# HydrogenSulfate/LFT

Measured on AMD Instinct MI355X. Metric: LF patches/sec (5x5 angRes, 32x32 LR, 4xSR), higher is better.
Workload: dtype bf16

## Files before the change

### lft_amd/_lib.py

```python
from __future__ import annotations

import ctypes
import os
import subprocess
from ctypes import POINTER, c_char_p, c_float, c_int, c_longlong, c_size_t, c_void_p

HERE = os.path.dirname(os.path.abspath(__file__))
CSRC = os.path.join(HERE, "csrc")
LIB_PATH = os.environ.get("LFT_LIB_PATH") or os.path.join(HERE, "liblft_hip.so")
SOURCES = ["lft_api.hip", "lft_common.cuh", "lft_kernels_a.cuh", "lft_kernels_b.cuh", "lft_train.cuh", "lft_train_host.cuh", "lft_metrics.cuh"]
ABI_VERSION = 5
STATUS_NONFINITE = 1001

PREC_F32, PREC_BF16, PREC_F16 = 0, 1, 2
MATH_F32, MATH_BF16X3, MATH_BF16X6 = 0, 1, 2
NUM_PARAMS = 78

_lib = None


class LftError(RuntimeError):
    pass


# ... 78 lines not shown
    "lft_spa_block_fwd": (c_int, [c_void_p, c_int, c_void_p, c_void_p, c_void_p, c_void_p, c_int, c_int, c_int, c_int, c_int, c_int, c_void_p]),
    "lft_upsample_fwd": (c_int, [c_void_p, c_void_p, c_void_p, c_void_p, c_void_p, c_int, c_int, c_int, c_int, c_int, c_int, c_void_p]),
    "lft_scene_counts": (c_int, [c_int, c_int, c_int, c_int, POINTER(c_int), POINTER(c_int)]),
    "lft_scene_divide": (c_int, [c_void_p, c_void_p, c_int, c_int, c_int, c_int, c_int, c_void_p]),
    "lft_scene_integrate": (c_int, [c_void_p, c_void_p, c_int, c_int, c_int, c_int, c_int, c_int, c_void_p]),
    "lft_train_tape_bytes": (c_int, [c_int, c_int, c_int, c_int, c_int, POINTER(c_size_t)]),
    "lft_train_grad_floats": (c_int, [c_int, POINTER(c_size_t)]),
    "lft_train_tape_offset": (c_int, [c_char_p, c_int, c_int, c_int, c_int, c_int, POINTER(c_size_t)]),
    "lft_train_forward": (c_int, [POINTER(c_void_p), c_int, c_void_p, c_void_p, c_void_p, c_int, c_int, c_int, c_int, c_int, c_int, c_void_p]),
    "lft_train_backward": (c_int, [POINTER(c_void_p), c_int, c_void_p, c_void_p, c_void_p, c_void_p, c_int, c_int, c_int, c_int, c_int, c_int, c_void_p]),
    "lft_train_backward_buckets": (c_int, [POINTER(c_void_p), c_int, c_void_p, c_void_p, c_void_p, c_void_p, c_int, c_int, c_int, c_int, c_int, c_int,
                                           c_void_p, c_void_p, c_void_p]),
    "lft_train_block_backward": (c_int, [POINTER(c_void_p), c_int, c_void_p, c_void_p, c_int, c_int, c_void_p, c_void_p, c_void_p,
                                         c_int, c_int, c_int, c_int, c_int, c_int, c_void_p]),
    "lft_train_grad_bucket": (c_int, [c_int, c_int, POINTER(c_size_t), POINTER(c_size_t)]),
    "lft_train_step_profiled": (c_int, [POINTER(c_void_p), c_int, c_void_p, c_void_p, c_void_p, c_void_p, c_void_p, c_int, c_int, c_int, c_int, c_int, c_int,
                                        c_void_p, c_int, POINTER(c_float), POINTER(c_char_p), POINTER(c_int)]),
    "lft_l1_loss": (c_int, [c_void_p, c_void_p, c_longlong, c_void_p, c_float, c_void_p, c_void_p, c_void_p]),
    "lft_adam_step": (c_int, [c_void_p, c_void_p, c_void_p, c_void_p, c_longlong, c_float, c_float, c_float, c_float, c_int, c_float, c_float, c_void_p]),
    "lft_view_metrics_scratch_bytes": (c_int, [c_int, c_int, c_int, c_int, POINTER(c_size_t)]),
    "lft_view_metrics": (c_int, [c_void_p, c_void_p, c_int, c_int, c_int, c_int, c_float, c_void_p, c_void_p, c_void_p, c_void_p]),
    "lft_debug_conv64": (c_int, [c_void_p, c_int, c_int, c_void_p, c_void_p, c_void_p, c_int, c_int, c_int, c_int, c_int, c_int, c_int, c_void_p]),
    "lft_mfma_selftest": (c_int, [c_void_p, c_void_p, c_void_p, c_void_p, c_void_p, c_int, c_void_p]),
}
EXPORTS = tuple(_SIGS)
TEST_EXPORTS = ("lft_debug_conv64", "lft_mfma_selftest")
BLOCK_UPSAMPLE, BLOCK_SPA, BLOCK_ANG, BLOCK_INIT = 0, 1, 2, 3
GRAD_BUCKETS = 3
BUCKET_FN = ctypes.CFUNCTYPE(c_int, c_void_p, c_int, c_size_t, c_size_t)


def lib() -> ctypes.CDLL:
    global _lib
    if _lib is None:
        if not os.path.exists(LIB_PATH):
            raise LftError(f"{LIB_PATH} is missing: the HIP extension has not been built "
                           "(run __graft_entry__.build()); there is no CPU fallback")
        L = ctypes.CDLL(LIB_PATH)
        L.lft_version.restype, L.lft_version.argtypes = c_int, []
        got = L.lft_version()
        if got != ABI_VERSION and not (os.environ.get("LFT_AB_ANY_ABI") == "1" and os.environ.get("LFT_LIB_PATH")):
            raise LftError(f"{LIB_PATH} reports ABI version {got}, this binding needs {ABI_VERSION}: rebuild it (__graft_entry__.build())")
        for name, (res, args) in _SIGS.items():
            if not hasattr(L, name) and got != ABI_VERSION:
                continue
            fn = getattr(L, name)
            fn.restype, fn.argtypes = res, args
        _lib = L
    return _lib
# ... 19 lines not shown
```

### lft_amd/csrc/lft_api.hip

```cpp
#include "../../include/lft_hip.h"
#include "../../include/lft_hip_test.h"
#include <hip/hip_runtime.h>
#include <stdint.h>

#include <cstdarg>
#include <cstdio>
#include <cmath>
#include <set>
#include <string>
#include <algorithm>
#include <utility>
#include <vector>

#ifndef LFT_TU
#define LFT_TU 0
#endif

namespace {
#include "lft_kernels_a.cuh"
#include "lft_kernels_b.cuh"
#include "lft_metrics.cuh"
#include "lft_train.cuh"
}

// ... 63 lines not shown
struct Dims {
    int B, A, V, h, w, hw, s, gp, gt, nchunk;
    long long ntok;
};

int make_dims(int B, int A, int h, int w, int s, int prec, Dims* d) {
    if (prec != LFT_PREC_F32 && prec != LFT_PREC_BF16 && prec != LFT_PREC_F16)
        return fail(LFT_ERR_ARG, "prec must be LFT_PREC_F32, LFT_PREC_BF16 or LFT_PREC_F16, got %d", prec);
    if (B < 1 || A < 1 || h < 1 || w < 1) return fail(LFT_ERR_SHAPE, "B, A, h, w must be positive (B=%d A=%d h=%d w=%d)", B, A, h, w);
    if (s != 2 && s != 4) return fail(LFT_ERR_SHAPE, "scale factor must be 2 or 4, got %d", s);
    if (A * A > 128) return fail(LFT_ERR_UNSUPPORTED, "angRes %d (A*A=%d views > 128) is not implemented in this build", A, A * A);
    if ((long long)B * A * A * h * w > (1LL << 27)) return fail(LFT_ERR_SHAPE, "too many tokens");
    d->B = B; d->A = A; d->V = A * A; d->h = h; d->w = w; d->hw = h * w; d->s = s;
    d->gp = (s + 2) * (s + 2); d->gt = (d->gp + 31) / 32; d->nchunk = 2 * s * s;
    d->ntok = (long long)B * d->V * d->hw;
    return 0;
}

constexpr int kFragsConv = 72, kFragsAng = 64, kFragsSpa1 = 240, kFragsSpa1NoQ = 208, kFragsSpa2 = 176;
inline int frags_up(const Dims& d) { return d.nchunk * (4 + 2 * d.gt); }

struct PackedLayout {
    size_t conv0_w, ln_ang[kLayers], ln_spa[kLayers], ang_pe, petok[kLayers], spa_pe_img;
    size_t s_conv[3], s_ang[kLayers], s_spa1[kLayers], s_spa2[kLayers], s_up, total;
};

PackedLayout packed_layout(const Dims& d, int prec) {
    const size_t esz = prec == LFT_PREC_F32 ? 4 : 2, fragb = 64 * 8 * esz;
    PackedLayout L;
    size_t o = 0;
    auto take = [&](size_t bytes) { size_t r = o; o = align256(o + bytes); return r; };
    L.conv0_w = take(576 * 4);
    for (int l = 0; l < kLayers; ++l) { L.ln_ang[l] = take(256 * 4); L.ln_spa[l] = take(512 * 4); }
    L.ang_pe = take((size_t)((d.V + 31) / 32) * 2048 * 4);
    for (int l = 0; l < kLayers; ++l) L.petok[l] = take((size_t)((d.hw + 32 * kNwSpa1 - 1) / (32 * kNwSpa1)) * kNwSpa1 * 4096 * esz);
    L.spa_pe_img = take((size_t)d.hw * 64 * esz);
    for (int i = 0; i < 3; ++i) L.s_conv[i] = take(kFragsConv * fragb);
    for (int l = 0; l < kLayers; ++l) {
        L.s_ang[l] = take(kFragsAng * fragb);
        L.s_spa1[l] = take(kFragsSpa1 * fragb);
        L.s_spa2[l] = take(kFragsSpa2 * fragb);
    }
    L.s_up = take((size_t)frags_up(d) * fragb);
    L.total = o;
    return L;
}

struct WorkLayout {
    size_t x0, feat, xa, xb, tok, q, k, v, o, g, status, total;
};
WorkLayout work_layout(const Dims& d, int prec) {
    const size_t esz = prec == LFT_PREC_F32 ? 4 : 2;
    WorkLayout W;
    size_t o = 0;
    auto take = [&](size_t bytes) { size_t r = o; o = align256(o + bytes); return r; };
    const size_t n = (size_t)d.ntok;
    W.x0 = take(n * 64 * esz); W.feat = take(n * 64 * esz); W.xa = take(n * 64 * esz); W.xb = take(n * 64 * esz);
    W.tok = take(n * 128 * esz); W.q = take(n * 128 * esz); W.k = take(n * 128 * esz); W.v = take(n * 128 * esz);
    W.o = take(n * 128 * esz);
    W.g = take(n * d.gp * 4);
    W.status = take(256);
    W.total = o;
    return W;
}

template <typename T> size_t lds_conv64(int w) { return WRing<T, kConv64Chunk, kNwConv>::LDS_BYTES + ConvIn<T, kNwConv>::bytes(w) + kNwConv * TileIO<2, T>::BYTES + kConvZeroRow; }
// ... 134 lines not shown
        {
            std::vector<PackOp> ops;
            ops.push_back(lin_op(q[4], 0, 128, 128, 0, 8, (sizeof(T) == 2 && tok_lane_major<T>(d)) ? 1 : 0, 1.0f));
            for (int c = 0; c < 4; ++c) {
                ops.push_back(lin_op(q[7], 64 * c, 64, 128, 0, 8, 1, 1.0f));
                ops.push_back(lin_op(q[8], 0, 128, 256, 64 * c, 4, 1, 1.0f));
            }
            ops.push_back(lin_op(q[9], 0, 64, 128, 0, 8, 1, 1.0f));
            if ((rc = run_pack<T>(ops, at<T>(packed, L.s_spa2[l]), kFragsSpa2, st))) return rc;
        }
        if ((rc = launch_spa1<T, true>((unsigned)((d.hw + 32 * kNwSpa1 - 1) / (32 * kNwSpa1)), at<T>(packed, L.spa_pe_img), at<T>(packed, L.s_spa1[l]), nullptr, nullptr,
                                       nullptr, nullptr, nullptr, nullptr, at<T>(packed, L.petok[l]), 1, d, st, nullptr))) return rc;
        LFT_LAUNCH_OK("k_spa1<pe>");
    }
    {
        std::vector<PackOp> ops;
        for (int c = 0; c < d.nchunk; ++c) {
            ops.push_back(lin_op(P[76], 32 * c, 32, 64, 0, 4, 1, 1.0f));
            PackOp m = lin_op(P[77], 0, d.gp, 0, 32 * c, 2, 1, 1.0f);
            m.kind = 1; m.s = d.s; m.ntiles = d.gt;
            ops.push_back(m);
        }
        if ((rc = run_pack<T>(ops, at<T>(packed, L.s_up), frags_up(d), st))) return rc;
    }
    return 0;
}

void launch_assemble(const float* lr, const float* g, float* out, int B, int A, int h, int w, int s, hipStream_t st, int gld = 0, unsigned* status = nullptr) {
    const dim3 tg((unsigned)((A * w + 7) / 8) * (unsigned)((A * h + 7) / 8) * (unsigned)B);
    if (!gld) gld = (s + 2) * (s + 2);
    if (s == 2) k_assemble_t<2><<<tg, 256, 0, st>>>(lr, g, out, B, A, h, w, gld, status);
    else k_assemble_t<4><<<tg, 256, 0, st>>>(lr, g, out, B, A, h, w, gld, status);
}

template <typename T>
int init_features(const void* packed, const PackedLayout& L, const float* lr, T* x0, T* ta, T* tb, T* feat, const Dims& d, hipStream_t st) {
    const int nimg = d.B * d.V, nwg = nimg * ((d.hw + 32 * kNwConv - 1) / (32 * kNwConv));
    const size_t lds = lds_conv64<T>(d.w);
    int rc;
    if ((rc = allow_lds(k_conv64<T, false>, lds, "k_conv64"))) return rc;
    if ((rc = allow_lds(k_conv64<T, true>, lds, "k_conv64"))) return rc;
    k_conv0<T><<<dim3((unsigned)((d.hw + kConv0Tok - 1) / kConv0Tok), (unsigned)nimg), 256, 0, st>>>(lr, at<float>(packed, L.conv0_w), x0, d.B, d.A, d.h, d.w);
    LFT_LAUNCH_OK("k_conv0");
    k_conv64<T, false><<<nwg, 64 * kNwConv, lds, st>>>(x0, ta, nullptr, at<T>(packed, L.s_conv[0]), nimg, d.h, d.w);
    LFT_LAUNCH_OK("k_conv64");
    k_conv64<T, false><<<nwg, 64 * kNwConv, lds, st>>>(ta, tb, nullptr, at<T>(packed, L.s_conv[1]), nimg, d.h, d.w);
// ... 90 lines not shown
    LFT_LAUNCH_OK("k_spa_attn");
    const unsigned nb = blocks_for(d.ntok, 32 * kNwSpa2);
    const bool lm = tok_lane_major<T>(d);
#define LFT_LAUNCH_SPA2(SKV, LMV, YLV)                                                                                      \
    do {                                                                                                                    \
        if ((rc = allow_lds(k_spa2<T, SKV, LMV, YLV>, lds_spa2<T>(), "k_spa2"))) return rc;                                 \
        k_spa2<T, SKV, LMV, YLV><<<nb, 64 * kNwSpa2, lds_spa2<T>(), st>>>(tok, o, at<T>(packed, L.s_spa2[l]), ln, skip, out, d.ntok, at<unsigned>(ws, W.status)); \
    } while (0)
    if (out_lm && !(skip && lm)) return fail(LFT_ERR_ARG, "internal: lane-major output needs the skip variant and full tiles");
    if (skip) { if (out_lm) LFT_LAUNCH_SPA2(true, true, true); else if (lm) LFT_LAUNCH_SPA2(true, true, false); else LFT_LAUNCH_SPA2(true, false, false); }
    else { if (lm) LFT_LAUNCH_SPA2(false, true, false); else LFT_LAUNCH_SPA2(false, false, false); }
#undef LFT_LAUNCH_SPA2
    LFT_LAUNCH_OK("k_spa2");
    return 0;
    }
}
template <typename T>
int spa_block(const void* packed, const PackedLayout& L, int l, const T* in, const T* skip, T* out, void* ws, const WorkLayout& W,
              const Dims& d, hipStream_t st, bool out_lm = false) {
    int rc;
    if ((rc = spa_part_a<T>(packed, L, l, in, ws, W, d, st))) return rc;
    return spa_part_b<T>(packed, L, l, skip, out, ws, W, d, st, out_lm);
}
template <typename T>
int upsample(const void* packed, const PackedLayout& L, const T* body, const float* lr, float* out, void* ws, const WorkLayout& W,
             const Dims& d, hipStream_t st, bool in_lm = false) {
    float* g = at<float>(ws, W.g);
    const unsigned nb = blocks_for(d.ntok, 32 * kNwUp);
    int rc;
#define LFT_LAUNCH_UP(GTV, LMV)                                                                                              \
    do {                                                                                                                    \
        if ((rc = allow_lds(k_up<T, GTV, LMV>, lds_up<T>(), "k_up"))) return rc;                                            \
        k_up<T, GTV, LMV><<<nb, 64 * kNwUp, lds_up<T>(), st>>>(body, at<T>(packed, L.s_up), g, d.ntok, d.nchunk, d.gp);     \
    } while (0)
    if (d.gt == 1) { if (in_lm) LFT_LAUNCH_UP(1, true); else LFT_LAUNCH_UP(1, false); }
    else { if (in_lm) LFT_LAUNCH_UP(2, true); else LFT_LAUNCH_UP(2, false); }
#undef LFT_LAUNCH_UP
    LFT_LAUNCH_OK("k_up");
    launch_assemble(lr, g, out, d.B, d.A, d.h, d.w, d.s, st, 0, at<unsigned>(ws, W.status));
    LFT_LAUNCH_OK("k_assemble");
    return 0;
}

template <typename T>
int forward_impl(const void* packed, const float* lr, float* out, void* ws, const Dims& d, int prec, hipStream_t st) {
    const PackedLayout L = packed_layout(d, prec);
    const WorkLayout W = work_layout(d, prec);
    T *x0 = at<T>(ws, W.x0), *feat = at<T>(ws, W.feat), *xa = at<T>(ws, W.xa), *xb = at<T>(ws, W.xb);
    int rc;
    if ((rc = init_features<T>(packed, L, lr, x0, xa, xb, feat, d, st))) return rc;
    const T* cur = feat;
    for (int l = 0; l < kLayers; ++l) {
        if ((rc = ang_block<T>(packed, L, l, cur, xa, d, st, at<unsigned>(ws, W.status)))) return rc;
        const bool last = l == kLayers - 1;
        if ((rc = spa_block<T>(packed, L, l, xa, last ? feat : nullptr, xb, ws, W, d, st, last && LFT_YLM && tok_lane_major<T>(d)))) return rc;
        cur = xb;
    }
    return upsample<T>(packed, L, xb, lr, out, ws, W, d, st, LFT_YLM && tok_lane_major<T>(d));
}

template <typename T>
int kernel_time_impl(const char* name, const void* packed, void* ws, const Dims& d, int prec, int reps, hipStream_t st, float* ms_out) {
    const PackedLayout L = packed_layout(d, prec);
    const WorkLayout W = work_layout(d, prec);
    T *x0 = at<T>(ws, W.x0), *feat = at<T>(ws, W.feat), *xa = at<T>(ws, W.xa), *xb = at<T>(ws, W.xb);
    const std::string k(name);
    auto once = [&]() -> int {
        if (k == "k_ang") return ang_block<T>(packed, L, 1, xb, xa, d, st, at<unsigned>(ws, W.status));
        if (k == "k_spa1") return spa_part_a<T>(packed, L, 1, xa, ws, W, d, st);
        if (k == "k_spa_b" || k == "k_spa_attn+k_spa2") return spa_part_b<T>(packed, L, 1, nullptr, xb, ws, W, d, st);
        if (k == "k_conv64") {
            const int nimg = d.B * d.V, nwg = nimg * ((d.hw + 32 * kNwConv - 1) / (32 * kNwConv));
            const size_t lds = lds_conv64<T>(d.w);
            int rc;
            if ((rc = allow_lds(k_conv64<T, false>, lds, "k_conv64"))) return rc;
            k_conv64<T, false><<<nwg, 64 * kNwConv, lds, st>>>(x0, feat, nullptr, at<T>(packed, L.s_conv[0]), nimg, d.h, d.w);
            LFT_LAUNCH_OK("k_conv64");
            return 0;
        }
        return fail(LFT_ERR_ARG, "lft_kernel_time: unknown kernel %s", name);
    };
    int rc;
    if ((rc = once())) return rc;
    hipEvent_t e0, e1;
    LFT_HIP_OK(hipEventCreate(&e0));
    LFT_HIP_OK(hipEventCreate(&e1));
    LFT_HIP_OK(hipEventRecord(e0, st));
    for (int i = 0; i < reps && !rc; ++i) rc = once();
    LFT_HIP_OK(hipEventRecord(e1, st));
    LFT_HIP_OK(hipEventSynchronize(e1));
    float ms = 0.0f;
    LFT_HIP_OK(hipEventElapsedTime(&ms, e0, e1));
    (void)hipEventDestroy(e0); (void)hipEventDestroy(e1);
// ... 134 lines not shown
}

int lft_spa_block_fwd(const void* packed, int layer, const void* act_in, const void* skip, void* act_out, void* workspace, int B, int A,
                      int h, int w, int s, int prec, void* stream) {
    Dims d; int rc;
    if (!packed || !act_in || !act_out || !workspace) return fail(LFT_ERR_ARG, "null pointer");
    if (layer < 0 || layer >= kLayers) return fail(LFT_ERR_ARG, "layer %d out of range", layer);
    if ((rc = make_dims(B, A, h, w, s, prec, &d))) return rc;
    const PackedLayout L = packed_layout(d, prec);
    const WorkLayout W = work_layout(d, prec);
    hipStream_t st = static_cast<hipStream_t>(stream);
    return LFT_BY_PREC(prec, spa_block<T>(packed, L, layer, static_cast<const T*>(act_in), static_cast<const T*>(skip),
                                          static_cast<T*>(act_out), workspace, W, d, st));
}

int lft_upsample_fwd(const void* packed, const void* act_in, const float* lr, float* out, void* workspace, int B, int A, int h, int w,
                     int s, int prec, void* stream) {
    Dims d; int rc;
    if (!packed || !act_in || !lr || !out || !workspace) return fail(LFT_ERR_ARG, "null pointer");
    if ((rc = make_dims(B, A, h, w, s, prec, &d))) return rc;
    const PackedLayout L = packed_layout(d, prec);
    const WorkLayout W = work_layout(d, prec);
    hipStream_t st = static_cast<hipStream_t>(stream);
    return LFT_BY_PREC(prec, upsample<T>(packed, L, static_cast<const T*>(act_in), lr, out, workspace, W, d, st));
}

int lft_debug_conv64(const void* packed, int which, int with_res, const void* in, const void* res, void* out, int B, int A, int h,
                     int w, int s, int prec, int extra_lds, void* stream) {
    Dims d; int rc;
    if (!packed || !in || !out || which < 0 || which > 2) return fail(LFT_ERR_ARG, "bad argument");
    if ((rc = make_dims(B, A, h, w, s, prec, &d))) return rc;
    const PackedLayout L = packed_layout(d, prec);
    hipStream_t st = static_cast<hipStream_t>(stream);
    const int nimg = d.B * d.V, nwg = nimg * ((d.hw + 32 * kNwConv - 1) / (32 * kNwConv));
    rc = LFT_BY_PREC(prec, [&]() -> int {
        const size_t lds = lds_conv64<T>(d.w) + extra_lds;
        int r;
        if ((r = allow_lds(k_conv64<T, false>, lds, "k_conv64"))) return r;
        if ((r = allow_lds(k_conv64<T, true>, lds, "k_conv64"))) return r;
        if (with_res) k_conv64<T, true><<<nwg, 64 * kNwConv, lds, st>>>((const T*)in, (T*)out, (const T*)res, at<T>(packed, L.s_conv[which]), nimg, d.h, d.w);
        else k_conv64<T, false><<<nwg, 64 * kNwConv, lds, st>>>((const T*)in, (T*)out, nullptr, at<T>(packed, L.s_conv[which]), nimg, d.h, d.w);
        return 0;
    }());
    if (rc) return rc;
    LFT_LAUNCH_OK("k_conv64");
    return 0;
}
// ... 227 lines not shown
```

### lft_amd/csrc/lft_common.cuh

```cuda
#pragma once
#include <hip/hip_runtime.h>
#include <stdint.h>
#include <utility>

typedef __bf16 bf16_t;
#ifndef LFT_PK
#define LFT_PK 1
#endif
#if LFT_PK
typedef float f32x2 __attribute__((ext_vector_type(2)));
__device__ __forceinline__ f32x2 p2_fma(f32x2 a, f32x2 b, f32x2 c) { return __builtin_elementwise_fma(a, b, c); }
#else
struct f32x2 {
    float v[2];
    __device__ __forceinline__ float& operator[](int i) { return v[i]; }
    __device__ __forceinline__ const float& operator[](int i) const { return v[i]; }
};
__device__ __forceinline__ f32x2 operator-(f32x2 a, f32x2 b) { return f32x2{a.v[0] - b.v[0], a.v[1] - b.v[1]}; }
__device__ __forceinline__ f32x2 operator+(f32x2 a, f32x2 b) { return f32x2{a.v[0] + b.v[0], a.v[1] + b.v[1]}; }
__device__ __forceinline__ f32x2 operator*(f32x2 a, f32x2 b) { return f32x2{a.v[0] * b.v[0], a.v[1] * b.v[1]}; }
__device__ __forceinline__ f32x2& operator+=(f32x2& a, f32x2 b) { a.v[0] += b.v[0]; a.v[1] += b.v[1]; return a; }
__device__ __forceinline__ f32x2 p2_fma(f32x2 a, f32x2 b, f32x2 c) { return f32x2{__builtin_fmaf(a.v[0], b.v[0], c.v[0]), __builtin_fmaf(a.v[1], b.v[1], c.v[1])}; }
#endif
typedef float f32x4 __attribute__((ext_vector_type(4)));
// ... 119 lines not shown
        LFT_VMCNT_CASE(32) LFT_VMCNT_CASE(33) LFT_VMCNT_CASE(34) LFT_VMCNT_CASE(35) LFT_VMCNT_CASE(36) LFT_VMCNT_CASE(37) LFT_VMCNT_CASE(38) LFT_VMCNT_CASE(39)
        LFT_VMCNT_CASE(40) LFT_VMCNT_CASE(41) LFT_VMCNT_CASE(42) LFT_VMCNT_CASE(43) LFT_VMCNT_CASE(44) LFT_VMCNT_CASE(45) LFT_VMCNT_CASE(46) LFT_VMCNT_CASE(47)
        LFT_VMCNT_CASE(48) LFT_VMCNT_CASE(49) LFT_VMCNT_CASE(50) LFT_VMCNT_CASE(51) LFT_VMCNT_CASE(52) LFT_VMCNT_CASE(53) LFT_VMCNT_CASE(54) LFT_VMCNT_CASE(55)
        LFT_VMCNT_CASE(56) LFT_VMCNT_CASE(57) LFT_VMCNT_CASE(58) LFT_VMCNT_CASE(59) LFT_VMCNT_CASE(60) LFT_VMCNT_CASE(61) LFT_VMCNT_CASE(62) LFT_VMCNT_CASE(63)
    }
}

LFT_DEV void wg_barrier_keep_vm() { asm volatile("s_waitcnt lgkmcnt(0)\n\ts_barrier" ::: "memory"); }
LFT_DEV void wg_barrier_keep_vm_lds_visible() {
    __builtin_amdgcn_s_waitcnt(0xC07F);
    asm volatile("s_barrier" ::: "memory");
}

#define LFT_NOTE_ASM_(kind, ring, slot) asm volatile("; LFT_NOTE " kind " ring=%0 slot=%1" :: "i"(ring), "i"(slot))
#define LFT_DMA_NOTE(kind, ring, slot) do { if (__builtin_constant_p(slot)) LFT_NOTE_ASM_(kind, ring, slot); } while (0)
constexpr int kNoteWRing = 0, kNoteWRingPipe = 1, kNoteKV = 2, kNoteConvIn = 3, kNoteAngW = 4;

template <typename T, int CH, int NW = 4>
struct WRing {
    static constexpr int NBUF = 3;
    static constexpr int FRAG_BYTES = 1024 * FragInfo<T>::PIECES;
    static constexpr int CHUNK_BYTES = CH * FRAG_BYTES;
    static constexpr int LDS_BYTES = NBUF * CHUNK_BYTES;
    static constexpr int PIECES_PER_WAVE = CH * FragInfo<T>::PIECES / NW;
    static_assert((CH * FragInfo<T>::PIECES) % NW == 0, "chunk must split over the workgroup's waves");
    static_assert(PIECES_PER_WAVE <= 12, "counted vmcnt immediates below cover up to 12 pieces per wave");
    const char* g;
    char* lds;
    int lane, wave, pos, nfrag;
    LFT_MEM void init(const T* stream, char* lds_base, int total_frags) {
        g = reinterpret_cast<const char*>(stream); lds = lds_base; nfrag = total_frags; pos = 0;
        lane = threadIdx.x & 63;
        wave = __builtin_amdgcn_readfirstlane(threadIdx.x >> 6);
        issue(0);
        issue(1);
    }
    LFT_MEM void issue(int c) {
        if (c * CH >= nfrag) return;
        const char* src = g + (size_t)c * CHUNK_BYTES;
        char* dst = lds + (c % NBUF) * CHUNK_BYTES;
        const int last = (nfrag - c * CH) * FragInfo<T>::PIECES - 1;
        LFT_DMA_NOTE("DMA", kNoteWRing, c % NBUF);
#pragma unroll
        for (int i = 0; i < PIECES_PER_WAVE; ++i) {
            const int piece = min(wave * PIECES_PER_WAVE + i, last);
            glds_piece(src + piece * 1024, dst + piece * 1024, lane);
        }
    }
    LFT_MEM void wait_landed(bool next_in_flight) { wait_vmcnt(next_in_flight ? PIECES_PER_WAVE : 0); }
    LFT_MEM Frag<T> next() {
        const int c = pos / CH, i = pos % CH;
        if (i == 0) {
            if (c > 0) LFT_DMA_NOTE("DONE", kNoteWRing, (c + NBUF - 1) % NBUF);
            wait_landed((c + 1) * CH < nfrag);
            wg_barrier_keep_vm();
            issue(c + 2);
            LFT_DMA_NOTE("USE", kNoteWRing, c % NBUF);
        }
        ++pos;
        return frag_from_pieces(lds + (c % NBUF) * CHUNK_BYTES + i * FRAG_BYTES, lane, T());
    }
};


template <typename T, int CH, int NW, int NBUF, int NFRAG>
struct WRingPipe {
    static constexpr int FRAG_BYTES = 1024 * FragInfo<T>::PIECES;
    static constexpr int CHUNK_BYTES = CH * FRAG_BYTES;
    static constexpr int LDS_BYTES = NBUF * CHUNK_BYTES;
    static constexpr int PIECES_PER_WAVE = CH * FragInfo<T>::PIECES / NW;
    static constexpr int NCHUNK = (NFRAG + CH - 1) / CH;
    static_assert((CH * FragInfo<T>::PIECES) % NW == 0, "chunk must split over the workgroup's waves");
    static_assert(PIECES_PER_WAVE * (NBUF - 1) <= 63, "counted vmcnt immediate");
    static constexpr int cmin(int a, int b) { return a < b ? a : b; }
    static constexpr int cmax(int a, int b) { return a > b ? a : b; }
    const char* g;
    char* lds;
    int lane, wave, split_slot, split_gap;
    Frag<T> fr0[CH], fr1[CH];
    LFT_MEM void setup(const T* stream, char* lds_base, int split_slot_ = NBUF, int split_gap_ = 0) {
        g = reinterpret_cast<const char*>(stream); lds = lds_base;
        split_slot = split_slot_; split_gap = split_gap_;
        lane = threadIdx.x & 63;
// ... 607 lines not shown
```

### lft_amd/csrc/lft_kernels_a.cuh

```cuda
#pragma once
#include "lft_common.cuh"

struct PackOp {
    const float* src;
    int kind, row0, nrows, ntiles, ld, kmul, kadd, k0, ksteps, kmap, frag0, s;
    float scale;
    int order;
};
__host__ __device__ __forceinline__ int wfrag_index(int OT, int KS, int ot, int ks) {
    const int g = ot >> 2, G = OT - 4 * g < 4 ? OT - 4 * g : 4;
    return 4 * g * KS + ks * G + (ot & 3);
}
__host__ __device__ __forceinline__ void wfrag_coords(int OT, int KS, int lf, int order, int& nt, int& ks) {
    if (!order) { nt = lf / KS; ks = lf % KS; return; }
    const int gl = (OT - 1) >> 2, g = lf / (4 * KS) < gl ? lf / (4 * KS) : gl, G = OT - 4 * g < 4 ? OT - 4 * g : 4, rem = lf - 4 * g * KS;
    ks = rem / G; nt = 4 * g + rem % G;
}
constexpr int LFT_PACK_MAXOPS = 40;
struct PackArgs {
    int nops;
    PackOp op[LFT_PACK_MAXOPS];
};

LFT_DEV float upm_entry(const float* __restrict__ w3, int n, int kk, int s) {
// ... 2 lines not shown
    const int dy = i - I, dx = j - J;
    if (dy < -1 || dy > 1 || dx < -1 || dx > 1) return 0.0f;
    return w3[c * 9 + (dy + 1) * 3 + (dx + 1)];
}

template <typename T>
__global__ __launch_bounds__(64) void k_pack(PackArgs args, T* __restrict__ dst) {
    const int f = blockIdx.x, lane = threadIdx.x, r = lane & 31, h = lane >> 5;
    int oi = 0;
    for (int i = 0; i < args.nops; ++i)
        if (f >= args.op[i].frag0) oi = i;
    const PackOp& op = args.op[oi];
    int nt, ks;
    wfrag_coords(op.ntiles, op.ksteps, f - op.frag0, op.order, nt, ks);
    const int n = 32 * nt + r;
#pragma unroll
    for (int j = 0; j < 8; ++j) {
        const int kk = op.k0 + 16 * ks + (op.kmap ? 8 * (j >> 2) + 4 * h + (j & 3) : 8 * h + j);
        float v = 0.0f;
        if (n < op.nrows) {
            if (op.kind == 0) v = op.scale * op.src[(size_t)(op.row0 + n) * op.ld + kk * op.kmul + op.kadd];
            else if (op.kind == 1) v = upm_entry(op.src, n, kk, op.s);
            else v = kk < (op.s + 2) * (op.s + 2) ? upm_entry(op.src, kk, n, op.s) : 0.0f;
        }
        if constexpr (sizeof(T) == 4) dst[(((size_t)f * 2 + (j >> 2)) * 64 + lane) * 4 + (j & 3)] = (T)v;
        else dst[((size_t)f * 64 + lane) * 8 + j] = (T)v;
    }
}

LFT_DEV float pe_value(int l, int c) {
    const int m = c & 31;
    const float g = (float)pow(10000.0, (double)(2 * m) / 64.0);
    const float p = (float)l / g;
    return (c < 32) ? (float)sin((double)p) : (float)cos((double)p);
}
template <typename T>
__global__ void k_pe_tables(float* __restrict__ ang_pe, T* __restrict__ spa_img, int V, int h, int w) {
    const int idx = blockIdx.x * blockDim.x + threadIdx.x;
    const int ntile = (V + 31) / 32;
    if (idx < ntile * 2048) {
        const int e = idx & 7, lane = (idx >> 3) & 63, k = (idx >> 9) & 3, ct = idx >> 11;
        const int view = ct * 32 + (lane & 31), nt = k >> 1, g = 2 * (k & 1) + (e >> 2);
        const int ch = 32 * nt + 8 * g + 4 * (lane >> 5) + (e & 3);
        ang_pe[idx] = view < V ? pe_value(view, ch) : 0.0f;
    }
    if (idx < h * w * 64) {
// ... 472 lines not shown
```

### lft_amd/csrc/lft_kernels_b.cuh

```cuda
#pragma once
#include "lft_common.cuh"
#include "lft_kernels_a.cuh"

#ifndef LFT_UP_CHUNK
#define LFT_UP_CHUNK 8
#endif
constexpr int kUpChunk = LFT_UP_CHUNK;
#ifndef LFT_SPA_CHUNK
#define LFT_SPA_CHUNK 16
#endif
#ifndef LFT_SPA_OCC
#define LFT_SPA_OCC 2
#endif
constexpr int kSpaChunk = LFT_SPA_CHUNK;
#ifndef LFT_NW_SPA1
#define LFT_NW_SPA1 4
#endif
#ifndef LFT_NW_SPA2
#define LFT_NW_SPA2 4
#endif
#ifndef LFT_NW_UP
#define LFT_NW_UP 8
#endif
constexpr int kNwSpa1 = LFT_NW_SPA1, kNwSpa2 = LFT_NW_SPA2, kNwUp = LFT_NW_UP;
// ... 696 lines not shown
        } else {
            const int a1 = Y / (h * S), a2 = X / (w * S);
            const float* view = lr + (size_t)b * MH * MW + (size_t)(a1 * h) * MW + a2 * w;
            v = bicubic_at(view, MW, h, w, Y - a1 * h * S, X - a2 * w * S, S);
        }
        const int ql = Yl / S + 1, qc = Xl / S + 1, i = Yl % S, j = Xl % S;
#pragma unroll
        for (int dy = -1; dy <= 1; ++dy) {
            const int I = i - S * dy;
            if (I < -1 || I > S) continue;
#pragma unroll
            for (int dx = -1; dx <= 1; ++dx) {
                const int J = j - S * dx;
                if (J < -1 || J > S) continue;
                v += gs[((ql + dy) * HL + qc + dx) * GP + (I + 1) * (S + 2) + (J + 1)];
            }
        }
        bad |= not_finite(v);
        out[((size_t)b * HR_H + Y) * HR_W + X] = v;
    }
    publish_status(status, bad);
}

LFT_DEV int reflect_idx(int i, int n) {
    i = i < 0 ? -i - 1 : i;
    return i >= n ? 2 * n - 1 - i : i;
}
__global__ __launch_bounds__(256) void k_scene_divide(const float* __restrict__ scene, float* __restrict__ patches,
                                                      int A, int h0, int w0, int patch, int stride, int nv) {
    const int X = blockIdx.x * 256 + threadIdx.x, Y = blockIdx.y, n = blockIdx.z;
    const int P = A * patch;
    if (X >= P) return;
    const int bdr = (patch - stride) / 2, ku = n / nv, kv = n - ku * nv;
    const int u = Y / patch, y = Y - u * patch, v = X / patch, x = X - v * patch;
    const int ey = ku * stride + y, ex = kv * stride + x;
    float val = 0.0f;
    if (ey < h0 + 2 * bdr && ex < w0 + 2 * bdr)
        val = scene[(size_t)(u * h0 + reflect_idx(ey - bdr, h0)) * (A * w0) + v * w0 + reflect_idx(ex - bdr, w0)];
    patches[((size_t)n * P + Y) * P + X] = val;
}
__global__ __launch_bounds__(256) void k_scene_integrate(const float* __restrict__ sub, float* __restrict__ out,
                                                         int A, int pz, int stride, int h0, int w0, int nv) {
    const int Xm = blockIdx.x * 256 + threadIdx.x, Ym = blockIdx.y;
    if (Xm >= A * w0) return;
    const int bdr = (pz - stride) / 2;
    const int u = Ym / h0, Y = Ym - u * h0, v = Xm / w0, X = Xm - v * w0;
// ... 49 lines not shown
```

Baseline: 9928.

## Fuse upsample conv, pixel-shuffle, and bicubic assemble into one tiled kernel

Adds a fused upsample kernel. Each workgroup computes the upsample GEMMs for an 8x32 LR tile, keeps the per-token 3x3 contribution grid in LDS, recomputes halo contributions from neighbouring tokens with separately packed edge weights, and writes HR output with bicubic LR interpolation added in place. This removes the global round trip of the intermediate grid buffer and the separate assemble kernel launch. The cost is redundant halo compute, a large LDS footprint and a new packed-weight region. The weight ring is also generalised to chunks that do not split evenly across waves.

After: 9756 (median of 6 runs). 0.983x the previous value.

```diff
diff --git a/lft_amd/_lib.py b/lft_amd/_lib.py
--- a/lft_amd/_lib.py
+++ b/lft_amd/_lib.py
@@ -124,9 +124,10 @@
     "lft_view_metrics": (c_int, [c_void_p, c_void_p, c_int, c_int, c_int, c_int, c_float, c_void_p, c_void_p, c_void_p, c_void_p]),
     "lft_debug_conv64": (c_int, [c_void_p, c_int, c_int, c_void_p, c_void_p, c_void_p, c_int, c_int, c_int, c_int, c_int, c_int, c_int, c_void_p]),
     "lft_mfma_selftest": (c_int, [c_void_p, c_void_p, c_void_p, c_void_p, c_void_p, c_int, c_void_p]),
+    "lft_debug_upsample": (c_int, [c_void_p, c_void_p, c_void_p, c_void_p, c_void_p, c_int, c_int, c_int, c_int, c_int, c_int, c_int, c_void_p]),
 }
 EXPORTS = tuple(_SIGS)
-TEST_EXPORTS = ("lft_debug_conv64", "lft_mfma_selftest")
+TEST_EXPORTS = ("lft_debug_conv64", "lft_mfma_selftest", "lft_debug_upsample")
 BLOCK_UPSAMPLE, BLOCK_SPA, BLOCK_ANG, BLOCK_INIT = 0, 1, 2, 3
 GRAD_BUCKETS = 3
 BUCKET_FN = ctypes.CFUNCTYPE(c_int, c_void_p, c_int, c_size_t, c_size_t)
diff --git a/lft_amd/csrc/lft_api.hip b/lft_amd/csrc/lft_api.hip
--- a/lft_amd/csrc/lft_api.hip
+++ b/lft_amd/csrc/lft_api.hip
@@ -109,7 +109,7 @@
 
 struct PackedLayout {
     size_t conv0_w, ln_ang[kLayers], ln_spa[kLayers], ang_pe, petok[kLayers], spa_pe_img;
-    size_t s_conv[3], s_ang[kLayers], s_spa1[kLayers], s_spa2[kLayers], s_up, total;
+    size_t s_conv[3], s_ang[kLayers], s_spa1[kLayers], s_spa2[kLayers], s_up, s_up_edge, total;
 };
 
 PackedLayout packed_layout(const Dims& d, int prec) {
@@ -129,6 +129,7 @@
         L.s_spa2[l] = take(kFragsSpa2 * fragb);
     }
     L.s_up = take((size_t)frags_up(d) * fragb);
+    L.s_up_edge = take((size_t)48 * d.s * fragb);
     L.total = o;
     return L;
 }
@@ -309,6 +310,8 @@
             ops.push_back(m);
         }
         if ((rc = run_pack<T>(ops, at<T>(packed, L.s_up), frags_up(d), st))) return rc;
+        k_pack_up_edge<T><<<48 * d.s, 64, 0, st>>>(P[76], P[77], at<T>(packed, L.s_up_edge), d.s);
+        LFT_LAUNCH_OK("k_pack_up_edge");
     }
     return 0;
 }
@@ -445,12 +448,28 @@
     if ((rc = spa_part_a<T>(packed, L, l, in, ws, W, d, st))) return rc;
     return spa_part_b<T>(packed, L, l, skip, out, ws, W, d, st, out_lm);
 }
+inline bool up_fused_ok(const Dims& d) { return d.h % kUpfRows == 0 && d.w % 32 == 0; }
 template <typename T>
 int upsample(const void* packed, const PackedLayout& L, const T* body, const float* lr, float* out, void* ws, const WorkLayout& W,
-             const Dims& d, hipStream_t st, bool in_lm = false) {
+             const Dims& d, hipStream_t st, bool in_lm, unsigned* status, bool fused = true) {
+    int rc;
+    if (fused && up_fused_ok(d)) {
+        const unsigned nwg = (unsigned)(d.B * d.V * (d.h / kUpfRows) * (d.w / 32));
+#define LFT_LAUNCH_UPF(SV, LMV)                                                                                              \
+        do {                                                                                                                \
+            constexpr size_t lds = UpFused<SV>::template lds_bytes<T>();                                                    \
+            if ((rc = allow_lds(k_up_fused<T, SV, LMV>, lds, "k_up_fused"))) return rc;                                      \
+            k_up_fused<T, SV, LMV><<<nwg, 64 * kUpfRows, lds, st>>>(body, at<T>(packed, L.s_up), at<T>(packed, L.s_up_edge), lr, out, \
+                                                                  d.A, d.h, d.w, status);                                    \
+        } while (0)
+        if (d.s == 2) { if (in_lm) LFT_LAUNCH_UPF(2, true); else LFT_LAUNCH_UPF(2, false); }
+        else { if (in_lm) LFT_LAUNCH_UPF(4, true); else LFT_LAUNCH_UPF(4, false); }
+#undef LFT_LAUNCH_UPF
+        LFT_LAUNCH_OK("k_up");
+        return 0;
+    }
     float* g = at<float>(ws, W.g);
     const unsigned nb = blocks_for(d.ntok, 32 * kNwUp);
-    int rc;
 #define LFT_LAUNCH_UP(GTV, LMV)                                                                                              \
     do {                                                                                                                    \
         if ((rc = allow_lds(k_up<T, GTV, LMV>, lds_up<T>(), "k_up"))) return rc;                                            \
@@ -460,7 +479,7 @@
     else { if (in_lm) LFT_LAUNCH_UP(2, true); else LFT_LAUNCH_UP(2, false); }
 #undef LFT_LAUNCH_UP
     LFT_LAUNCH_OK("k_up");
-    launch_assemble(lr, g, out, d.B, d.A, d.h, d.w, d.s, st, 0, at<unsigned>(ws, W.status));
+    launch_assemble(lr, g, out, d.B, d.A, d.h, d.w, d.s, st, 0, status);
     LFT_LAUNCH_OK("k_assemble");
     return 0;
 }
@@ -479,7 +498,7 @@
         if ((rc = spa_block<T>(packed, L, l, xa, last ? feat : nullptr, xb, ws, W, d, st, last && LFT_YLM && tok_lane_major<T>(d)))) return rc;
         cur = xb;
     }
-    return upsample<T>(packed, L, xb, lr, out, ws, W, d, st, LFT_YLM && tok_lane_major<T>(d));
+    return upsample<T>(packed, L, xb, lr, out, ws, W, d, st, LFT_YLM && tok_lane_major<T>(d), at<unsigned>(ws, W.status));
 }
 
 template <typename T>
@@ -492,6 +511,7 @@
         if (k == "k_ang") return ang_block<T>(packed, L, 1, xb, xa, d, st, at<unsigned>(ws, W.status));
         if (k == "k_spa1") return spa_part_a<T>(packed, L, 1, xa, ws, W, d, st);
         if (k == "k_spa_b" || k == "k_spa_attn+k_spa2") return spa_part_b<T>(packed, L, 1, nullptr, xb, ws, W, d, st);
+        if (k == "k_up") return upsample<T>(packed, L, xb, at<float>(ws, W.k), at<float>(ws, W.q), ws, W, d, st, LFT_YLM && tok_lane_major<T>(d), nullptr);
         if (k == "k_conv64") {
             const int nimg = d.B * d.V, nwg = nimg * ((d.hw + 32 * kNwConv - 1) / (32 * kNwConv));
             const size_t lds = lds_conv64<T>(d.w);
@@ -672,7 +692,19 @@
     const PackedLayout L = packed_layout(d, prec);
     const WorkLayout W = work_layout(d, prec);
     hipStream_t st = static_cast<hipStream_t>(stream);
-    return LFT_BY_PREC(prec, upsample<T>(packed, L, static_cast<const T*>(act_in), lr, out, workspace, W, d, st));
+    return LFT_BY_PREC(prec, upsample<T>(packed, L, static_cast<const T*>(act_in), lr, out, workspace, W, d, st, false, at<unsigned>(workspace, W.status)));
+}
+
+int lft_debug_upsample(const void* packed, const void* act_in, const float* lr, float* out, void* workspace, int B, int A, int h, int w,
+                       int s, int prec, int fused, void* stream) {
+    Dims d; int rc;
+    if (!packed || !act_in || !lr || !out || !workspace) return fail(LFT_ERR_ARG, "null pointer");
+    if ((rc = make_dims(B, A, h, w, s, prec, &d))) return rc;
+    const PackedLayout L = packed_layout(d, prec);
+    const WorkLayout W = work_layout(d, prec);
+    hipStream_t st = static_cast<hipStream_t>(stream);
+    return LFT_BY_PREC(prec, upsample<T>(packed, L, static_cast<const T*>(act_in), lr, out, workspace, W, d, st, false,
+                                         at<unsigned>(workspace, W.status), fused != 0));
 }
 
 int lft_debug_conv64(const void* packed, int which, int with_res, const void* in, const void* res, void* out, int B, int A, int h,
diff --git a/lft_amd/csrc/lft_common.cuh b/lft_amd/csrc/lft_common.cuh
--- a/lft_amd/csrc/lft_common.cuh
+++ b/lft_amd/csrc/lft_common.cuh
@@ -165,8 +165,8 @@
     static constexpr int FRAG_BYTES = 1024 * FragInfo<T>::PIECES;
     static constexpr int CHUNK_BYTES = CH * FRAG_BYTES;
     static constexpr int LDS_BYTES = NBUF * CHUNK_BYTES;
-    static constexpr int PIECES_PER_WAVE = CH * FragInfo<T>::PIECES / NW;
-    static_assert((CH * FragInfo<T>::PIECES) % NW == 0, "chunk must split over the workgroup's waves");
+    static constexpr bool EVEN = (CH * FragInfo<T>::PIECES) % NW == 0;
+    static constexpr int PIECES_PER_WAVE = (CH * FragInfo<T>::PIECES + NW - 1) / NW;
     static_assert(PIECES_PER_WAVE <= 12, "counted vmcnt immediates below cover up to 12 pieces per wave");
     const char* g;
     char* lds;
@@ -182,7 +182,8 @@
         if (c * CH >= nfrag) return;
         const char* src = g + (size_t)c * CHUNK_BYTES;
         char* dst = lds + (c % NBUF) * CHUNK_BYTES;
-        const int last = (nfrag - c * CH) * FragInfo<T>::PIECES - 1;
+        int last = (nfrag - c * CH) * FragInfo<T>::PIECES - 1;
+        if constexpr (!EVEN) last = min(last, CH * FragInfo<T>::PIECES - 1);
         LFT_DMA_NOTE("DMA", kNoteWRing, c % NBUF);
 #pragma unroll
         for (int i = 0; i < PIECES_PER_WAVE; ++i) {
@@ -191,17 +192,19 @@
         }
     }
     LFT_MEM void wait_landed(bool next_in_flight) { wait_vmcnt(next_in_flight ? PIECES_PER_WAVE : 0); }
+    LFT_MEM void enter(int c) {
+        if (c > 0) LFT_DMA_NOTE("DONE", kNoteWRing, (c + NBUF - 1) % NBUF);
+        wait_landed((c + 1) * CH < nfrag);
+        wg_barrier_keep_vm();
+        issue(c + 2);
+        LFT_DMA_NOTE("USE", kNoteWRing, c % NBUF);
+    }
+    LFT_MEM Frag<T> at(int c, int i) const { return frag_from_pieces(lds + (c % NBUF) * CHUNK_BYTES + i * FRAG_BYTES, lane, T()); }
     LFT_MEM Frag<T> next() {
         const int c = pos / CH, i = pos % CH;
-        if (i == 0) {
-            if (c > 0) LFT_DMA_NOTE("DONE", kNoteWRing, (c + NBUF - 1) % NBUF);
-            wait_landed((c + 1) * CH < nfrag);
-            wg_barrier_keep_vm();
-            issue(c + 2);
-            LFT_DMA_NOTE("USE", kNoteWRing, c % NBUF);
-        }
+        if (i == 0) enter(c);
         ++pos;
-        return frag_from_pieces(lds + (c % NBUF) * CHUNK_BYTES + i * FRAG_BYTES, lane, T());
+        return at(c, i);
     }
 };
 
diff --git a/lft_amd/csrc/lft_kernels_a.cuh b/lft_amd/csrc/lft_kernels_a.cuh
--- a/lft_amd/csrc/lft_kernels_a.cuh
+++ b/lft_amd/csrc/lft_kernels_a.cuh
@@ -48,6 +48,30 @@
             if (op.kind == 0) v = op.scale * op.src[(size_t)(op.row0 + n) * op.ld + kk * op.kmul + op.kadd];
             else if (op.kind == 1) v = upm_entry(op.src, n, kk, op.s);
             else v = kk < (op.s + 2) * (op.s + 2) ? upm_entry(op.src, kk, n, op.s) : 0.0f;
+        }
+        if constexpr (sizeof(T) == 4) dst[(((size_t)f * 2 + (j >> 2)) * 64 + lane) * 4 + (j & 3)] = (T)v;
+        else dst[((size_t)f * 64 + lane) * 8 + j] = (T)v;
+    }
+}
+
+LFT_DEV int up_edge_channel(int side, int e, int s) {
+    const int c = e / s, m = e % s;
+    const int i = side == 0 ? s - 1 : side == 1 ? 0 : m, j = side == 0 || side == 1 ? m : side == 2 ? s - 1 : 0;
+    return c * s * s + i * s + j;
+}
+template <typename T>
+__global__ __launch_bounds__(64) void k_pack_up_edge(const float* __restrict__ wu, const float* __restrict__ w3, T* __restrict__ dst, int s) {
+    const int f = blockIdx.x, lane = threadIdx.x, r = lane & 31, h = lane >> 5;
+    const int side = f / (12 * s), t = (f / 6) % (2 * s), k = f % 6;
+#pragma unroll
+    for (int j = 0; j < 8; ++j) {
+        const int kl = 8 * (j >> 2) + 4 * h + (j & 3);
+        float v = 0.0f;
+        if (k < 4) {
+            v = wu[(size_t)up_edge_channel(side, 32 * t + r, s) * 64 + 16 * k + kl];
+        } else if (r < s + 2) {
+            const int I = side == 0 ? s : side == 1 ? -1 : r - 1, J = side < 2 ? r - 1 : side == 2 ? s : -1;
+            v = upm_entry(w3, (I + 1) * (s + 2) + (J + 1), up_edge_channel(side, 32 * t + 16 * (k - 4) + kl, s), s);
         }
         if constexpr (sizeof(T) == 4) dst[(((size_t)f * 2 + (j >> 2)) * 64 + lane) * 4 + (j & 3)] = (T)v;
         else dst[((size_t)f * 64 + lane) * 8 + j] = (T)v;
diff --git a/lft_amd/csrc/lft_kernels_b.cuh b/lft_amd/csrc/lft_kernels_b.cuh
--- a/lft_amd/csrc/lft_kernels_b.cuh
+++ b/lft_amd/csrc/lft_kernels_b.cuh
@@ -742,6 +742,205 @@
     publish_status(status, bad);
 }
 
+constexpr int kUpfRows = 8;
+template <int S> struct UpFused {
+    static constexpr int GP = (S + 2) * (S + 2), GT = (GP + 31) / 32, FPI = 4 + 2 * GT;
+    static constexpr int IPC = 2, CH = IPC * FPI, NIT = 2 * S * S;
+    static constexpr int EN = S + 2;
+    static constexpr int EDGE_FRAGS = 4 * 2 * S * 6;
+    static constexpr int TLY = kUpfRows + 4, TLX = 32 + 4;
+    template <typename T> static constexpr int eg_offset() {
+        return WRing<T, CH, kUpfRows>::LDS_BYTES > kUpfRows * 32 * GP * 4 ? WRing<T, CH, kUpfRows>::LDS_BYTES : kUpfRows * 32 * GP * 4;
+    }
+    template <typename T> static constexpr int lds_bytes() { return eg_offset<T>() + (4 * 2 * EN * 32 + TLY * TLX) * 4; }
+};
+template <typename T, bool LM>
+LFT_DEV void load_x_tok(const T* __restrict__ X, long long tok, bool ok, int lane, f32x16 (&a)[2]) {
+    const int hh = lane >> 5;
+    if constexpr (LM) {
+        const T* base = X + (tok & ~31LL) * 64;
+        const int ln = 32 * hh + (int)(tok & 31);
+#pragma unroll
+        for (int nt = 0; nt < 2; ++nt)
+#pragma unroll
+            for (int k = 0; k < 2; ++k) {
+                const char* src = reinterpret_cast<const char*>(base + ((size_t)(nt * 2 + k) * 64 + ln) * 8);
+                if constexpr (sizeof(T) == 2) {
+                    const auto v = __builtin_bit_cast(typename H16<T>::v8, load_raw16(src));
+#pragma unroll
+                    for (int j = 0; j < 8; ++j) a[nt][8 * k + j] = ok ? (float)v[j] : 0.0f;
+                } else {
+                    const f32x4 lo = __builtin_bit_cast(f32x4, load_raw16(src)), hi = __builtin_bit_cast(f32x4, load_raw16(src + 16));
+#pragma unroll
+                    for (int j = 0; j < 4; ++j) { a[nt][8 * k + j] = ok ? lo[j] : 0.0f; a[nt][8 * k + 4 + j] = ok ? hi[j] : 0.0f; }
+                }
+            }
+    } else {
+        load_acc<2, T>(X + tok * 64, ok, hh, a);
+    }
+}
+template <typename T, int S, bool XLM>
+__global__ __launch_bounds__(64 * kUpfRows) void k_up_fused(const T* __restrict__ X, const T* __restrict__ ws, const T* __restrict__ we,
+                                                           const float* __restrict__ lr, float* __restrict__ out, int A, int h, int w,
+                                                           unsigned* __restrict__ status) {
+    using P = UpFused<S>;
+    constexpr int R = kUpfRows, GP = P::GP, GT = P::GT, FPI = P::FPI, IPC = P::IPC, EN = P::EN, TLX = P::TLX, TLY = P::TLY;
+    using Ring = WRing<T, P::CH, R>;
+    extern __shared__ __attribute__((aligned(16))) char smem[];
+    float* gs = reinterpret_cast<float*>(smem);
+    float* eg = reinterpret_cast<float*>(smem + P::template eg_offset<T>());
+    float* lt = eg + 4 * 2 * EN * 32;
+    constexpr int kEgFloat = P::template eg_offset<T>() / 4;
+    const int lane = threadIdx.x & 63, r = lane & 31, hh = lane >> 5, wave = threadIdx.x >> 6;
+    const int tpr = w / 32, tpc = h / R, V = A * A, hw = h * w, MH = A * h, MW = A * w;
+    const int bid = xcd_tile(blockIdx.x, gridDim.x);
+    const int tx = bid % tpr, ty = (bid / tpr) % tpc, im = bid / (tpr * tpc);
+    const int b = im / V, v = im - b * V, vy = v / A, vx = v - vy * A;
+    const int x0 = tx * 32, y0 = ty * R, my0 = vy * h + y0, mx0 = vx * w + x0;
+    LFT_STAMP(0);
+    f32x16 x[2], xh[2];
+    load_x_tok<T, XLM>(X, (long long)im * hw + (long long)(y0 + wave) * w + x0 + r, true, lane, x);
+    const int side = wave >> 1, half = wave & 1;
+    const int my = side == 0 ? my0 - 1 : side == 1 ? my0 + R : my0 - 1 + r;
+    const int mx = side < 2 ? mx0 + r : side == 2 ? mx0 - 1 : mx0 + 32;
+    const bool hok = my >= 0 && my < MH && mx >= 0 && mx < MW && (side < 2 || r < R + 2);
+    {
+        const int myc = min(max(my, 0), MH - 1), mxc = min(max(mx, 0), MW - 1), hvy = myc / h, hvx = mxc / w;
+        const long long htok = ((long long)(b * V + hvy * A + hvx)) * hw + (long long)(myc - hvy * h) * w + (mxc - hvx * w);
+        load_x_tok<T, XLM>(X, htok, hok, lane, xh);
+    }
+    float tap = 0.0f;
+    if (threadIdx.x < TLY * TLX) {
+        const int rr = threadIdx.x / TLX, cc = threadIdx.x - rr * TLX;
+        const int yy = min(max(my0 - 2 + rr, vy * h), vy * h + h - 1), xx = min(max(mx0 - 2 + cc, vx * w), vx * w + w - 1);
+        tap = lr[(size_t)b * MH * MW + (size_t)yy * MW + xx];
+    }
+    Ring ring;
+    ring.init(ws, smem, P::NIT * FPI);
+    if (threadIdx.x < TLY * TLX) lt[threadIdx.x] = tap;
+    LFT_STAMP(1);
+    {
+        Frag<T> hf[4];
+        acc_frags<2, T>(xh, hf);
+        f32x16 ge[1];
+        zero_acc<1>(ge);
+        const int f0 = (side * 2 * S + half * S) * 6;
+#pragma unroll
+        for (int t = 0; t < S; ++t) {
+            Frag<T> wf[6];
+#pragma unroll
+            for (int k = 0; k < 6; ++k) wf[k] = load_wfrag(we, f0 + 6 * t + k, lane);
+            f32x16 u[1];
+            zero_acc<1>(u);
+#pragma unroll
+            for (int ks = 0; ks < 4; ++ks) mma(wf[ks], hf[ks], u[0]);
+#pragma unroll
+            for (int i = 0; i < 16; ++i) u[0][i] = lrelu02_fast(u[0][i]);
+            Frag<T> uf[2];
+            acc_frags<1, T>(u, uf);
+            mma(wf[4], uf[0], ge[0]);
+            mma(wf[5], uf[1], ge[0]);
+        }
+        float* egw = eg + (side * 2 + half) * EN * 32 + r;
+#pragma unroll
+        for (int i = 0; i < 16; ++i) {
+            const int n = acc_row(i, hh);
+            if (n < EN) egw[n * 32] = ge[0][i];
+        }
+    }
+    LFT_STAMP(2);
+    Frag<T> xf[4];
+    acc_frags<2, T>(x, xf);
+    f32x16 g[GT];
+    zero_acc<GT>(g);
+#pragma unroll 1
+    for (int c = 0; c < P::NIT / IPC; ++c) {
+        ring.enter(c);
+        f32x16 u[IPC];
+        zero_acc<IPC>(u);
+#pragma unroll
+        for (int ks = 0; ks < 4; ++ks)
+#pragma unroll
+            for (int it = 0; it < IPC; ++it) mma(ring.at(c, it * FPI + ks), xf[ks], u[it]);
+#pragma unroll
+        for (int it = 0; it < IPC; ++it) {
+#pragma unroll
+            for (int i = 0; i < 16; ++i) u[it][i] = lrelu02_fast(u[it][i]);
+            const Frag<T> uf[2] = {acc_to_frag(u[it], 0, T()), acc_to_frag(u[it], 1, T())};
+#pragma unroll
+            for (int nt = 0; nt < GT; ++nt)
+#pragma unroll
+                for (int ks = 0; ks < 2; ++ks) mma(ring.at(c, it * FPI + 4 + 2 * nt + ks), uf[ks], g[nt]);
+        }
+    }
+    LFT_STAMP(3);
+    wg_barrier_keep_vm();
+    for (int k = threadIdx.x; k < 4 * EN * 32; k += 64 * R) {
+        float* e = eg + (k / (EN * 32)) * 2 * EN * 32 + k % (EN * 32);
+        e[0] = e[0] + e[EN * 32];
+    }
+    {
+        float* gw = gs + (wave * 32 + r) * GP;
+#pragma unroll
+        for (int nt = 0; nt < GT; ++nt)
+#pragma unroll
+            for (int grp = 0; grp < 4; ++grp) {
+                const int base = 32 * nt + 8 * grp + 4 * hh;
+                if (base < GP) *reinterpret_cast<f32x4*>(gw + base) = f32x4{g[nt][4 * grp], g[nt][4 * grp + 1], g[nt][4 * grp + 2], g[nt][4 * grp + 3]};
+            }
+    }
+    wg_barrier_keep_vm();
+    LFT_STAMP(4);
+    constexpr int TSX = 32 * S, NPIX = R * S * TSX;
+    static_assert((64 * R) % TSX == 0, "every thread keeps its column");
+    const int Yl0 = threadIdx.x / TSX, Xl0 = threadIdx.x - Yl0 * TSX;
+    float cy[4], cx[4];
+    const float sy = ((float)Yl0 + 0.5f) / (float)S - 0.5f, sx = ((float)Xl0 + 0.5f) / (float)S - 0.5f;
+    const float fy = floorf(sy), fx = floorf(sx);
+    cubic_coef(sy - fy, cy);
+    cubic_coef(sx - fx, cx);
+    const int ry = (int)fy - Yl0 / S, rx = (int)fx - Xl0 / S;
+    const int HR_W = MW * S;
+    float* ob = out + ((size_t)b * MH * S + (size_t)my0 * S) * HR_W + (size_t)mx0 * S;
+    unsigned bad = 0;
+    for (int idx = threadIdx.x; idx < NPIX; idx += 64 * R) {
+        const int Yl = idx / TSX, Xl = idx - Yl * TSX;
+        const float* t0 = lt + (2 + Yl / S + ry - 1) * TLX + (2 + Xl / S + rx - 1);
+        float acc = 0.0f;
+#pragma unroll
+        for (int a = 0; a < 4; ++a) {
+            float row = 0.0f;
+#pragma unroll
+            for (int bb = 0; bb < 4; ++bb) row += cx[bb] * t0[a * TLX + bb];
+            acc += cy[a] * row;
+        }
+        float val = acc;
+        const int ql = Yl / S, qc = Xl / S, i = Yl % S, j = Xl % S;
+        float gv[9];
+        bool use[9];
+#pragma unroll
+        for (int dy = -1; dy <= 1; ++dy)
+#pragma unroll
+            for (int dx = -1; dx <= 1; ++dx) {
+                const int I = i - S * dy, J = j - S * dx, q = (dy + 1) * 3 + dx + 1;
+                use[q] = I >= -1 && I <= S && J >= -1 && J <= S;
+                const int nr = ql + dy, nc = qc + dx;
+                const bool inside = nr >= 0 && nr < R && nc >= 0 && nc < 32;
+                const int sd = nc < 0 ? 2 : nc >= 32 ? 3 : nr < 0 ? 0 : 1;
+                const int ln = sd >= 2 ? nr + 1 : nc, n = sd >= 2 ? I + 1 : J + 1;
+                const int ofs = !use[q] ? 0 : inside ? (nr * 32 + nc) * GP + (I + 1) * (S + 2) + (J + 1) : kEgFloat + (sd * 2 * EN + n) * 32 + ln;
+                gv[q] = gs[ofs];
+            }
+#pragma unroll
+        for (int q = 0; q < 9; ++q)
+            if (use[q]) val += gv[q];
+        bad |= not_finite(val);
+        ob[(size_t)Yl * HR_W + Xl] = val;
+    }
+    LFT_STAMP(5);
+    publish_status(status, bad);
+}
+
 LFT_DEV int reflect_idx(int i, int n) {
     i = i < 0 ? -i - 1 : i;
     return i >= n ? 2 * n - 1 - i : i;
```
